# facebookresearch/iris

Hardware: AMD Instinct MI355X
Metric: bake_shading throughput (shading samples/s: secondary rays traced and shaded) (higher is better)
Workload: dtype f32; 1 GPU; bake_shading train-view sequence (15 views evenly spaced among 32 cameras on a circle, one view per step), 1920x1080, SPP=128 per lobe, lobes=[0, 1, 2, 3, 4, 5, 6] (0=diffuse,1-6=specular), synthetic room seed=1 1000990 triangles, SLF H=256, Philox uniforms; pixels_per_view=2073600

## Files before the change

### iris_amd/csrc/iris_bake.h

```cpp
#pragma once
#include "iris_tile.h"

namespace iris {

struct BakeArgs {
    SceneDev sc; EmitDev em; SlfDev slf;
    const float* pos; const float* nrm; const float* wo;
    const float* u2; const int32_t* pix_id;
    int64_t P; int spp; uint64_t seed; uint32_t stream_id; float rough;
    float* out0; float* out1; int64_t* tri_next;
    int64_t* src_next;
    unsigned long long* stats;
    uint32_t* stack_ovf;
    float4* scratch;
    unsigned int* tile_counter;
    int tile_px;
};

#ifndef IRIS_TILE_RAYS
#define IRIS_TILE_RAYS 5120
#endif
constexpr int kTileRays = IRIS_TILE_RAYS;

__device__ __forceinline__ void reduce_geometry(int spp, int& lpp, int& ppw, int& rounds) {
    if (spp >= 64) { lpp = 64; ppw = 1; rounds = (spp + 63) >> 6; }
    else if ((spp & (spp - 1)) == 0) { lpp = spp; ppw = 64 / spp; rounds = 1; }
    else { lpp = 64; ppw = 1; rounds = 1; }
}

struct RayOut { float r0, g0, b0, r1, g1, b1; };

template <bool SPEC>
__device__ __forceinline__ void sample_dir(const BakeArgs& a, float u0, float u1, f3 n, f3 w, f3 t, f3 b, f3& wi, float& g0, float& g1) {
    g0 = 1.f; g1 = 0.f;
    if (SPEC) {
        wi = specular_sampler(u0, u1, a.rough, w, n, t, b);
        SpecW sw = specular_weights(wi, w, n, a.rough, false);
        g0 = sw.g0; g1 = sw.g1;
    } else {
        wi = diffuse_sampler(u0, u1, n, t, b);
    }
}
template <bool SPEC>
__device__ __forceinline__ void sample_lobe(const BakeArgs& a, int64_t p, int s, f3 n, f3 w, f3 t, f3 b, uint64_t base, f3& wi, float& g0, float& g1) {
    float u0, u1;
    if (a.u2) { const float* up = a.u2 + (p * a.spp + s) * 2; u0 = up[0]; u1 = up[1]; }
    else {
        uint32_t s_lo = (uint32_t)a.seed, s_hi = (uint32_t)(a.seed >> 32);
        asm volatile("" : "+s"(s_lo), "+s"(s_hi));
        philox_u2(((uint64_t)s_hi << 32) | s_lo, base + (uint64_t)s, a.stream_id, u0, u1);
    }
    sample_dir<SPEC>(a, u0, u1, n, w, t, b, wi, g0, g1);
}

template <bool SPEC, bool COUNT, int LAYOUT, int LDS_DEPTH = kStackLds, bool GLOBAL_OVF = false>
__device__ __forceinline__ RayOut trace_shade(const BakeArgs& a, int64_t p, int s, f3 x, f3 wi, float g0, float g1, uint32_t* lds_stack,
                                              TraceStats* ts, uint32_t& n_rays, uint32_t* ovf = nullptr) {
    f3 o = mk3(x.x + kRayEps * wi.x, x.y + kRayEps * wi.y, x.z + kRayEps * wi.z);
    const uint32_t steps0 = COUNT ? ts->nodes + ts->tris : 0;
    Hit h = trace_bvh4<LAYOUT, COUNT, LDS_DEPTH, GLOBAL_OVF>(a.sc, o, wi, lds_stack, ts, ovf);
    if (COUNT) {
        n_rays++;
        uint32_t mine = ts->nodes + ts->tris - steps0, mx = mine;
        for (int m = 1; m < 64; m <<= 1) mx = max(mx, (uint32_t)__shfl_xor((int)mx, m));
        if (first_active_lane()) ts->max_steps64 += (unsigned long long)mx * 64ull;
    }
    f3 pn = mk3(0.f, 0.f, 0.f);
    int64_t tri = -1;
    if (h.slot >= 0) {
        f3 p0, p1, p2;
        hit_vertices(a.sc, h, p0, p1, p2);
        pn = hit_position(h, p0, p1, p2);
        tri = h.id;
    }
    if (a.tri_next) a.tri_next[p * a.spp + s] = tri;
    float epdf; bool vn; int src;
    f3 Le = eval_emitter1(a.em, a.slf, pn, tri, true, 1.0f, 0.0f, epdf, vn, src);
    if (a.src_next) a.src_next[p * a.spp + s] = src;
    RayOut r;
    if (SPEC) { r.r0 = Le.x * g0; r.g0 = Le.y * g0; r.b0 = Le.z * g0; r.r1 = Le.x * g1; r.g1 = Le.y * g1; r.b1 = Le.z * g1; }
    else { r.r0 = Le.x; r.g0 = Le.y; r.b0 = Le.z; r.r1 = r.g1 = r.b1 = 0.f; }
    return r;
}

__device__ __forceinline__ bool dead_samples_skippable(const BakeArgs& a) { return !a.tri_next && !a.src_next; }

template <bool SPEC, bool COUNT, int LAYOUT, int LDS_DEPTH = kStackLds, bool GLOBAL_OVF = false>
__device__ __forceinline__ RayOut shade_sample(const BakeArgs& a, int64_t p, int s, f3 x, f3 n, f3 w, f3 t, f3 b, uint64_t base,
                                               uint32_t* lds_stack, TraceStats* ts, uint32_t& n_rays, uint32_t* ovf = nullptr) {
    f3 wi; float g0, g1;
    sample_lobe<SPEC>(a, p, s, n, w, t, b, base, wi, g0, g1);
    if (SPEC && !COUNT && dead_samples_skippable(a) && g0 == 0.f && g1 == 0.f) return RayOut{0.f, 0.f, 0.f, 0.f, 0.f, 0.f};
    return trace_shade<SPEC, COUNT, LAYOUT, LDS_DEPTH, GLOBAL_OVF>(a, p, s, x, wi, g0, g1, lds_stack, ts, n_rays, ovf);
}

template <bool COUNT>
__device__ __forceinline__ void flush_stats(const BakeArgs& a, const TraceStats& ts, uint32_t n_rays) {
    if (COUNT) {
        uint32_t v[8] = {n_rays, ts.nodes, ts.tris, ts.node_iters, ts.leaf_iters, ts.sp_gt8, ts.sp_gt12, ts.sp_gt16};
        for (int k = 0; k < 8; ++k) {
            uint32_t x = v[k];
            for (int m = 1; m < 64; m <<= 1) x += __shfl_xor(x, m);
            if ((threadIdx.x & 63) == 0) atomicAdd(a.stats + k, (unsigned long long)x);
        }
        uint32_t w[2] = {ts.drain_nodes, ts.drain_node_iters};
        for (int k = 0; k < 2; ++k) {
            uint32_t x = w[k];
            for (int m = 1; m < 64; m <<= 1) x += __shfl_xor(x, m);
            if ((threadIdx.x & 63) == 0) atomicAdd(a.stats + 9 + k, (unsigned long long)x);
        }
        uint32_t tp[4] = {ts.top21, ts.top85, ts.top341, ts.top1365};
        for (int k = 0; k < 4; ++k) {
            uint32_t x = tp[k];
            for (int m = 1; m < 64; m <<= 1) x += __shfl_xor(x, m);
            if ((threadIdx.x & 63) == 0) atomicAdd(a.stats + 11 + k, (unsigned long long)x);
        }
        uint32_t sh[5] = {ts.shared_iters, ts.shared_lanes, ts.shared_all_iters, ts.slow_push_iters, ts.shared_path_iters};
        for (int k = 0; k < 5; ++k) {
            uint32_t x = sh[k];
            for (int m = 1; m < 64; m <<= 1) x += __shfl_xor(x, m);
            if ((threadIdx.x & 63) == 0) atomicAdd(a.stats + 15 + k, (unsigned long long)x);
        }
        unsigned long long y = ts.max_steps64;
        for (int m = 1; m < 64; m <<= 1) y += __shfl_xor(y, m);
        if ((threadIdx.x & 63) == 0) atomicAdd(a.stats + 8, y);
    }
}

template <bool SPEC, bool COUNT, int LAYOUT>
__global__ __launch_bounds__(kBlock) void bake_kernel(BakeArgs a) {
    __shared__ uint32_t s_stack[kStackLds * kBlock];
    const int lane = threadIdx.x & 63;
    const int spp = a.spp;
    int lpp, ppw, rounds;
    reduce_geometry(spp, lpp, ppw, rounds);
    const int sub = lane / lpp, sl = lane - sub * lpp;
    const int64_t n_groups = (a.P + ppw - 1) / ppw;
    const int64_t wave0 = ((int64_t)blockIdx.x * kBlock + threadIdx.x) >> 6;
    const int64_t n_waves = ((int64_t)gridDim.x * kBlock) >> 6;
    const float inv_spp = 1.0f / (float)spp;
    TraceStats ts;
    uint32_t n_rays = 0;

    for (int64_t g = wave0; g < n_groups; g += n_waves) {
        const int64_t p = g * ppw + sub;
        const bool pvalid = p < a.P;
        f3 x = mk3(0.f, 0.f, 0.f), n = mk3(0.f, 0.f, 1.f), w = mk3(0.f, 0.f, 1.f), t, b;
        uint64_t base = 0;
        if (pvalid) {
            x = ld3(a.pos + p * 3); n = ld3(a.nrm + p * 3);
            if (SPEC) w = ld3(a.wo + p * 3);
            base = (uint64_t)(a.pix_id ? (int64_t)a.pix_id[p] : p) * (uint64_t)spp;
        }
        normal_space(n, t, b);
        float a0x = 0.f, a0y = 0.f, a0z = 0.f, a1x = 0.f, a1y = 0.f, a1z = 0.f;
        for (int r = 0; r < rounds; ++r) {
            const int s = r * 64 + sl;
            if (pvalid && s < spp) {
                RayOut o = shade_sample<SPEC, COUNT, LAYOUT>(a, p, s, x, n, w, t, b, base, s_stack + threadIdx.x, &ts, n_rays);
                a0x += o.r0; a0y += o.g0; a0z += o.b0;
                if (SPEC) { a1x += o.r1; a1y += o.g1; a1z += o.b1; }
            }
        }
        for (int m = 1; m < lpp; m <<= 1) {
            a0x += __shfl_xor(a0x, m); a0y += __shfl_xor(a0y, m); a0z += __shfl_xor(a0z, m);
            if (SPEC) { a1x += __shfl_xor(a1x, m); a1y += __shfl_xor(a1y, m); a1z += __shfl_xor(a1z, m); }
        }
        if (pvalid && sl == 0) {
            st3(a.out0 + p * 3, mk3(a0x * inv_spp, a0y * inv_spp, a0z * inv_spp));
            if (SPEC) st3(a.out1 + p * 3, mk3(a1x * inv_spp, a1y * inv_spp, a1z * inv_spp));
        }
    }
    flush_stats<COUNT>(a, ts, n_rays);
}

#ifndef IRIS_TILE_WAVES
#define IRIS_TILE_WAVES 7
#endif
#ifndef IRIS_TILE_STACK
#define IRIS_TILE_STACK 12
#endif

template <bool SPEC, bool COUNT, int LAYOUT, int TILE_STACK>
__device__ __forceinline__ void tile_body(const BakeArgs& a, int64_t p0, int np, float4* res, uint16_t* s_sorted, uint32_t* s_stack, int* s_chunk,
                                          uint32_t* ovf, TraceStats& ts, uint32_t& n_rays) {
    const int tid = threadIdx.x, lane = tid & 63, wave = tid >> 6;
    const int spp = a.spp;
    float2* res_g = reinterpret_cast<float2*>(res + kTileRays);
    int lpp, ppw, rounds;
    reduce_geometry(spp, lpp, ppw, rounds);
    const int sub = lane / lpp, sl = lane - sub * lpp;
    const float inv_spp = 1.0f / (float)spp;
    const int nr = np * spp;
    const bool resolve = !a.em.emit_ord && !a.tri_next;
    const bool skip_dead = dead_samples_skippable(a);

    const uint32_t spp_m = spp > 1 ? (uint32_t)(0x100000000ull / (uint64_t)(uint32_t)spp) + 1u : 0u;
    auto div_spp = [&](int r) -> int { return spp > 1 ? (int)__umulhi((uint32_t)r, spp_m) : r; };

    constexpr int kFrameOff = (kTileRays + 2 * 256 * 4) / 4, kFramePx = (TILE_STACK * kBlock - kFrameOff) / 6;
    float* s_frames = reinterpret_cast<float*>(s_stack) + kFrameOff;
    const bool frames = np <= kFramePx;
    if (frames) {
        for (int pl = tid; pl < np; pl += kBlock) {
            f3 t, b;
            normal_space(ld3(a.nrm + (p0 + pl) * 3), t, b);
            float* f = s_frames + pl * 6;
            f[0] = t.x; f[1] = t.y; f[2] = t.z; f[3] = b.x; f[4] = b.y; f[5] = b.z;
        }
        __syncthreads();
    }

    tile_sort_trace<LAYOUT, COUNT, kTileRays, TILE_STACK, true, SPEC && !COUNT>(
        a.sc, nr, s_sorted, s_stack, s_chunk, ovf, ts,
        [&](int r) -> uint32_t {
            const int pl = div_spp(r), s = r - pl * spp;
            const int64_t p = p0 + pl;
            const f3 n = ld3(a.nrm + p * 3), w = SPEC ? ld3(a.wo + p * 3) : mk3(0.f, 0.f, 1.f);
            const uint64_t base = (uint64_t)(a.pix_id ? (int64_t)a.pix_id[p] : p) * (uint64_t)spp;
            f3 t, b;
            if (frames) { const float* f = s_frames + pl * 6; t = mk3(f[0], f[1], f[2]); b = mk3(f[3], f[4], f[5]); }
            else normal_space(n, t, b);
            f3 wi; float g0, g1;
            sample_lobe<SPEC>(a, p, s, n, w, t, b, base, wi, g0, g1);
            if (SPEC) res_g[r] = make_float2(g1, g0);
            const bool dead = SPEC && !COUNT && skip_dead && g0 == 0.f && g1 == 0.f;
            res[r] = dead ? make_float4(0.f, 0.f, __int_as_float(resolve ? 0 : -1), __int_as_float(resolve ? -2 : 0)) : make_float4(wi.x, wi.y, wi.z, 0.f);
            return dead ? kDeadRay : dir_bin(wi);
        },
        [&](int r, f3& o, f3& d) {
            const int64_t p = p0 + div_spp(r);
            o = ld3(a.pos + p * 3);
            const float4 qa = res[r];
            d = mk3(qa.x, qa.y, qa.z);
        },
        [&](f3& o, f3& d) { o = mk3(o.x + kRayEps * d.x, o.y + kRayEps * d.y, o.z + kRayEps * d.z); },
        [&](int r, const Hit& h) {
            if (resolve) {
                float4 q = make_float4(0.f, 0.f, 0.f, __int_as_float(-2));
                if (h.slot >= 0) {
                    const float4* tr = a.sc.tris + (int64_t)h.slot * 4;
                    const float4 tx = tr[0], ty = tr[1], tz = tr[2];
                    const float ow = tr[3].x;
                    const f3 pn = hit_position(h, mk3(tx.x, ty.x, tz.x), mk3(tx.y, ty.y, tz.y), mk3(tx.z, ty.z, tz.z));
                    q = make_float4(pn.x, pn.y, pn.z, ow);
                }
                res[r] = q;
            } else
            res[r] = make_float4(h.u, h.v, __int_as_float(h.slot), 0.f);
            if (COUNT) n_rays++; }
        );

    const int n_groups = (np + ppw - 1) / ppw;
    IRIS_PHASE_BEGIN();
    for (int g = wave; g < n_groups; g += kBlock / 64) {
        const int pl = g * ppw + sub;
        const bool pvalid = pl < np;
        float a0x = 0.f, a0y = 0.f, a0z = 0.f, a1x = 0.f, a1y = 0.f, a1z = 0.f;
        if (resolve) {
            for (int rr = 0; rr < rounds; rr += 2) {
                const int s0 = rr * 64 + sl, s1 = s0 + 64;
                const bool ok0 = pvalid && s0 < spp, ok1 = pvalid && rr + 1 < rounds && s1 < spp;
                float4 q0 = make_float4(0.f, 0.f, 0.f, __int_as_float(-2)), q1 = q0;
                float2 w0 = make_float2(0.f, 0.f), w1 = w0;
                if (ok0) { q0 = res[pl * spp + s0]; if (SPEC) w0 = res_g[pl * spp + s0]; }
                if (ok1) { q1 = res[pl * spp + s1]; if (SPEC) w1 = res_g[pl * spp + s1]; }
                const int o0 = __float_as_int(q0.w), o1 = __float_as_int(q1.w);
                int j0 = -1, j1 = -1;
                if (o0 == -1) j0 = slf_index(a.slf, mk3(q0.x, q0.y, q0.z));
                if (o1 == -1) j1 = slf_index(a.slf, mk3(q1.x, q1.y, q1.z));
                float4 r0 = make_float4(0.f, 0.f, 0.f, 0.f), r1 = r0;
                if (o0 >= 0 || j0 >= 0) r0 = *(o0 >= 0 ? a.em.radiance + o0 : a.slf.radiance + j0);
                if (o1 >= 0 || j1 >= 0) r1 = *(o1 >= 0 ? a.em.radiance + o1 : a.slf.radiance + j1);
                if (ok0) {
                    const float z = o0 >= 0 ? -0.f : 0.f;
                    const f3 Le = mk3(z + r0.x, z + r0.y, z + r0.z);
                    if (a.src_next) a.src_next[(p0 + pl) * spp + s0] = o0 >= 0 ? -2 - o0 : j0;
                    if (SPEC) { a0x += Le.x * w0.y; a0y += Le.y * w0.y; a0z += Le.z * w0.y; a1x += Le.x * w0.x; a1y += Le.y * w0.x; a1z += Le.z * w0.x; }
                    else { a0x += Le.x; a0y += Le.y; a0z += Le.z; }
                }
                if (ok1) {
                    const float z = o1 >= 0 ? -0.f : 0.f;
                    const f3 Le = mk3(z + r1.x, z + r1.y, z + r1.z);
                    if (a.src_next) a.src_next[(p0 + pl) * spp + s1] = o1 >= 0 ? -2 - o1 : j1;
                    if (SPEC) { a0x += Le.x * w1.y; a0y += Le.y * w1.y; a0z += Le.z * w1.y; a1x += Le.x * w1.x; a1y += Le.y * w1.x; a1z += Le.z * w1.x; }
                    else { a0x += Le.x; a0y += Le.y; a0z += Le.z; }
                }
            }
        } else
        for (int rr = 0; rr < rounds; ++rr) {
            const int s = rr * 64 + sl;
            if (pvalid && s < spp) {
                const float4 qa = res[pl * spp + s];
                Hit h; h.u = qa.x; h.v = qa.y; h.slot = __float_as_int(qa.z); h.t = 0.f; h.id = 0;
                f3 pn = mk3(0.f, 0.f, 0.f);
                int64_t tri = -1;
                int ord_rec = -1;
                if (h.slot >= 0) {
                    const float4* tr = a.sc.tris + (int64_t)h.slot * 4;
                    const float4 tx = tr[0], ty = tr[1], tz = tr[2];
                    if (!a.em.emit_ord) ord_rec = __float_as_int(tr[3].x);
                    pn = hit_position(h, mk3(tx.x, ty.x, tz.x), mk3(tx.y, ty.y, tz.y), mk3(tx.z, ty.z, tz.z));
                    tri = __float_as_int(tx.w);
                }
                if (a.tri_next) a.tri_next[(p0 + pl) * spp + s] = tri;
                float epdf; bool vn; int src;
                const f3 Le = eval_emitter1(a.em, a.slf, pn, tri, true, 1.0f, 0.0f, epdf, vn, src, ord_rec);
                if (a.src_next) a.src_next[(p0 + pl) * spp + s] = src;
                if (SPEC) {
                    const float2 qb = res_g[pl * spp + s];
                    a0x += Le.x * qb.y; a0y += Le.y * qb.y; a0z += Le.z * qb.y;
                    a1x += Le.x * qb.x; a1y += Le.y * qb.x; a1z += Le.z * qb.x;
                } else { a0x += Le.x; a0y += Le.y; a0z += Le.z; }
            }
        }
        for (int m = 1; m < lpp; m <<= 1) {
            a0x += __shfl_xor(a0x, m); a0y += __shfl_xor(a0y, m); a0z += __shfl_xor(a0z, m);
            if (SPEC) { a1x += __shfl_xor(a1x, m); a1y += __shfl_xor(a1y, m); a1z += __shfl_xor(a1z, m); }
        }
        if (pvalid && sl == 0) {
            const int64_t p = p0 + pl;
            st3(a.out0 + p * 3, mk3(a0x * inv_spp, a0y * inv_spp, a0z * inv_spp));
            if (SPEC) st3(a.out1 + p * 3, mk3(a1x * inv_spp, a1y * inv_spp, a1z * inv_spp));
        }
    }
    IRIS_PHASE_MARK(3);
}

constexpr int kTileChunk = 64;
__device__ __forceinline__ long long claim_tile(unsigned int* counters, long long n_tiles) {
    constexpr int kChunk = kTileChunk;
    const long long n_chunks = (n_tiles + kChunk - 1) / kChunk;
    for (int k = 0; k < 8; ++k) {
        const int x = ((int)blockIdx.x + k) & 7;
        const long long per = (n_chunks + 7 - x) / 8;
        for (;;) {
            const unsigned int c = atomicAdd(counters + x, 1u);
            const long long ch = (long long)(c / kChunk);
            if (ch >= per) break;
            const long long t = (ch * 8 + x) * kChunk + (c % kChunk);
            if (t < n_tiles) return t;
        }
    }
    return n_tiles;
}

template <bool SPEC, bool COUNT, int LAYOUT>
__global__ __launch_bounds__(kBlock, COUNT ? 4 : IRIS_TILE_WAVES) void bake_tile_kernel(BakeArgs a) {
    constexpr int kTileStack = IRIS_TILE_STACK;
    __shared__ uint16_t s_sorted[kTileRays];
    __shared__ uint32_t s_stack[kTileStack * kBlock];
    __shared__ int s_tile, s_chunk;
    static_assert(kTileStack * kBlock * 4 >= kTileRays + 2 * 256 * 4, "stack region too small to alias the sort keys");
    const int tid = threadIdx.x;
    constexpr int NC = SPEC ? 2 : 1;
    float4* res = a.scratch + (size_t)blockIdx.x * kTileRays * NC;
    uint32_t* ovf = a.stack_ovf + (size_t)blockIdx.x * (kStackCapacity - kTileStack) * kBlock;
    const int64_t n_tiles = (a.P + a.tile_px - 1) / a.tile_px;
    TraceStats ts;
    uint32_t n_rays = 0;
    for (;;) {
        __syncthreads();
        if (tid == 0) { s_tile = (int)claim_tile(a.tile_counter, n_tiles); s_chunk = 0; }
        (s_stack + kTileRays / 4)[tid] = 0;
        __syncthreads();
        const int64_t tile = s_tile;
        if (tile >= n_tiles) break;
        const int64_t p0 = (int64_t)tile * a.tile_px;
        tile_body<SPEC, COUNT, LAYOUT, kTileStack>(a, p0, (int)min((int64_t)a.tile_px, a.P - p0), res, s_sorted, s_stack, &s_chunk, ovf, ts, n_rays);
    }
    flush_stats<COUNT>(a, ts, n_rays);
}

constexpr int kMaxLobes = 8;
struct ViewLobe { float rough; int spp; uint32_t stream_id; int spec; int tile_px; int tiles_per_span; float* out0; float* out1; };
struct ViewArgs {
    BakeArgs base;
    int n_lobes;
    int span_px;
    long long n_tiles;
    ViewLobe lobe[kMaxLobes];
};

template <int LAYOUT>
__global__ __launch_bounds__(kBlock, IRIS_TILE_WAVES) void bake_view_kernel(ViewArgs v) {
    constexpr int kTileStack = IRIS_TILE_STACK;
    __shared__ uint16_t s_sorted[kTileRays];
    __shared__ uint32_t s_stack[kTileStack * kBlock];
    __shared__ int s_tile, s_chunk;
    static_assert(kTileStack * kBlock * 4 >= kTileRays + 2 * 256 * 4, "stack region too small to alias the sort keys");
    const int tid = threadIdx.x;
    float4* res = v.base.scratch + (size_t)blockIdx.x * kTileRays * 2;
    uint32_t* ovf = v.base.stack_ovf + (size_t)blockIdx.x * (kStackCapacity - kTileStack) * kBlock;
    for (;;) {
        __syncthreads();
        if (tid == 0) { s_tile = (int)claim_tile(v.base.tile_counter, v.n_tiles); s_chunk = 0; }
        (s_stack + kTileRays / 4)[tid] = 0;
        __syncthreads();
        const long long vt = s_tile;
        if (vt >= v.n_tiles) break;
        const long long g = vt / kTileChunk, q = g >> 3;
        const int j = (int)(vt % kTileChunk), l = (int)(q % v.n_lobes);
        const int64_t span0 = ((q / v.n_lobes) * 8 + (g & 7)) * (int64_t)v.span_px;
        const int64_t p0 = span0 + (int64_t)j * v.lobe[l].tile_px;
        if (j >= v.lobe[l].tiles_per_span || p0 >= v.base.P) continue;
        const int np = (int)min((int64_t)v.lobe[l].tile_px, min(v.base.P, span0 + v.span_px) - p0);
        BakeArgs a = v.base;
        a.spp = v.lobe[l].spp; a.rough = v.lobe[l].rough; a.stream_id = v.lobe[l].stream_id; a.tile_px = v.lobe[l].tile_px;
        a.out0 = v.lobe[l].out0; a.out1 = v.lobe[l].out1; a.u2 = nullptr; a.tri_next = nullptr; a.src_next = nullptr;
        TraceStats ts; uint32_t n_rays = 0;
        if (v.lobe[l].spec) tile_body<true, false, LAYOUT, kTileStack>(a, p0, np, res, s_sorted, s_stack, &s_chunk, ovf, ts, n_rays);
        else tile_body<false, false, LAYOUT, kTileStack>(a, p0, np, res, s_sorted, s_stack, &s_chunk, ovf, ts, n_rays);
    }
}

}
```

### iris_amd/csrc/iris_tile.h

```cpp
#pragma once
#include "iris_trace.h"

namespace iris {

#ifndef IRIS_PRIO_A
#define IRIS_PRIO_A 0
#endif
#ifndef IRIS_PRIO_C
#define IRIS_PRIO_C 3
#endif
#ifndef IRIS_PRIO_D
#define IRIS_PRIO_D 0
#endif

__device__ __forceinline__ uint32_t dir_bin(f3 d) {
    const float ax = fabsf(d.x), ay = fabsf(d.y), az = fabsf(d.z);
    const float inv = __builtin_amdgcn_rcpf(ax + ay + az + 1e-30f);
    const float a = ax * inv, b = ay * inv;
    const float v = b * __builtin_amdgcn_rcpf(1.f - a + 1e-30f);
    const int iu = min(7, (int)(a * 8.f)), iv0 = min(3, (int)(v * 4.f));
    const int iv = (iu & 1) ? 3 - iv0 : iv0;
    const uint32_t oct = (d.x < 0.f ? 1u : 0u) | (d.y < 0.f ? 2u : 0u) | (d.z < 0.f ? 4u : 0u);
    return (oct << 5) | ((uint32_t)iu << 2) | (uint32_t)iv;
}

#ifdef IRIS_PHASE_TIMING
__device__ unsigned long long g_phase_cycles[8];
#define IRIS_PHASE_BEGIN() unsigned long long t_phase_ = clock64()
#define IRIS_PHASE_MARK(k) do { if (threadIdx.x == 0) { const unsigned long long t_ = clock64(); atomicAdd(&g_phase_cycles[k], t_ - t_phase_); t_phase_ = t_; } } while (0)
#else
#define IRIS_PHASE_BEGIN()
#define IRIS_PHASE_MARK(k)
#endif

constexpr uint32_t kDeadRay = 256u;
template <int LAYOUT, bool COUNT, int CAP, int TILE_STACK, bool GLOBAL_OVF, bool SKIP_DEAD = false, class PhaseA, class FetchRay, class Prepare, class Retire>
__device__ __forceinline__ void tile_sort_trace(const SceneDev& sc, int nr, uint16_t* s_sorted, uint32_t* s_stack, int* s_chunk, uint32_t* ovf,
                                                TraceStats& ts, PhaseA phase_a, FetchRay fetch_ray, Prepare prepare, Retire retire) {
    static_assert(TILE_STACK * kBlock * 4 >= CAP + 2 * 256 * 4, "stack region too small to alias the sort keys");
    static_assert(!SKIP_DEAD || CAP <= 32 * kBlock, "one bit per ray of a thread");
    uint8_t* s_keys = reinterpret_cast<uint8_t*>(s_stack);
    uint32_t* s_hist = s_stack + CAP / 4;
    uint32_t* s_cur = s_hist + 256;
    const int tid = threadIdx.x, lane = tid & 63, wave = tid >> 6;
    IRIS_PHASE_BEGIN();
    __builtin_amdgcn_s_setprio(IRIS_PRIO_A);
    uint32_t dead = 0;
    if (SKIP_DEAD) {
        uint32_t bit = 1u;
        for (int r = tid; r < nr; r += kBlock, bit <<= 1) {
            const uint32_t key = phase_a(r);
            if (key == kDeadRay) dead |= bit;
            else { s_keys[r] = (uint8_t)key; atomicAdd(&s_hist[key], 1u); }
        }
    } else
    for (int r = tid; r < nr; r += kBlock) {
        const uint32_t key = phase_a(r);
        s_keys[r] = (uint8_t)key;
        atomicAdd(&s_hist[key], 1u);
    }
    __syncthreads();
    IRIS_PHASE_MARK(0);
    if (wave == 0) {
        uint32_t c0 = s_hist[lane * 4], c1 = s_hist[lane * 4 + 1], c2 = s_hist[lane * 4 + 2], c3 = s_hist[lane * 4 + 3];
        uint32_t tot = c0 + c1 + c2 + c3, inc = tot;
        for (int m = 1; m < 64; m <<= 1) { uint32_t v = __shfl_up(inc, m); if (lane >= m) inc += v; }
        uint32_t ex = inc - tot;
        if (SKIP_DEAD) {
            const uint32_t first = (uint32_t)nr - (uint32_t)__builtin_amdgcn_readlane((int)inc, 63);
            ex += first;
            if (lane == 0) *s_chunk = (int)first;
        }
        s_cur[lane * 4] = ex; s_cur[lane * 4 + 1] = ex + c0; s_cur[lane * 4 + 2] = ex + c0 + c1; s_cur[lane * 4 + 3] = ex + c0 + c1 + c2;
    }
    __syncthreads();
    if (SKIP_DEAD) {
        for (int r = tid; r < nr; r += kBlock, dead >>= 1) {
            if (dead & 1u) continue;
            const uint32_t pos = atomicAdd(&s_cur[s_keys[r]], 1u);
            s_sorted[pos] = (uint16_t)r;
        }
    } else
    for (int r = tid; r < nr; r += kBlock) {
        const uint32_t pos = atomicAdd(&s_cur[s_keys[r]], 1u);
        s_sorted[pos] = (uint16_t)r;
    }
    __syncthreads();
    IRIS_PHASE_MARK(1);
    {
        int my_r = 0;
        auto fetch = [&](f3& o, f3& d) -> bool {
            const unsigned long long m = __ballot(1);
            int base = 0;
            if (lane == __ffsll((long long)m) - 1) base = atomicAdd(s_chunk, __popcll(m));
            base = __builtin_amdgcn_readfirstlane(base);
            const int i = base + (int)__builtin_amdgcn_mbcnt_hi((uint32_t)(m >> 32), __builtin_amdgcn_mbcnt_lo((uint32_t)m, 0u));
            if (i >= nr) return false;
            my_r = s_sorted[i];
            fetch_ray(my_r, o, d);
            return true;
        };
        auto ret = [&](const Hit& h) { retire(my_r, h); };
        __builtin_amdgcn_s_setprio(IRIS_PRIO_C);
        uint32_t tid_c = threadIdx.x;
        asm volatile("" : "+v"(tid_c));
        SceneDev sc_c = sc;
        asm volatile("" : "+s"(sc_c.nodes), "+s"(sc_c.tris), "+s"(sc_c.oct_stride));
        trace_stream<LAYOUT, COUNT, TILE_STACK, GLOBAL_OVF>(sc_c, s_stack + tid_c, tid_c, ovf, &ts, fetch, prepare, ret);
        __builtin_amdgcn_s_setprio(IRIS_PRIO_D);
        IRIS_PHASE_MARK(4);
    }
    __syncthreads();
    IRIS_PHASE_MARK(2);
}

}
```

Before: 10510 Mrays/s.

## Reload kernel arguments per phase to shrink live scalar register state

Restructures tile_body so each phase (sampling, tracing, shading) reloads only the kernel arguments it needs straight from the kernarg segment via fresh pointers, instead of holding a full BakeArgs copy live across the whole tile. The goal is to cut SGPR/VGPR pressure and spills across the long trace loop, which could allow more waves or a tighter inner loop. Adds lobe-source abstractions for the single-lobe and multi-lobe view kernels. The cost is repeated scalar loads from kernarg memory at each phase entry, and the changes depend on compiler register allocation behaving as intended.

```diff
diff --git a/iris_amd/csrc/iris_bake.h b/iris_amd/csrc/iris_bake.h
--- a/iris_amd/csrc/iris_bake.h
+++ b/iris_amd/csrc/iris_bake.h
@@ -30,8 +30,8 @@
 
 struct RayOut { float r0, g0, b0, r1, g1, b1; };
 
-template <bool SPEC>
-__device__ __forceinline__ void sample_dir(const BakeArgs& a, float u0, float u1, f3 n, f3 w, f3 t, f3 b, f3& wi, float& g0, float& g1) {
+template <bool SPEC, class A>
+__device__ __forceinline__ void sample_dir(const A& a, float u0, float u1, f3 n, f3 w, f3 t, f3 b, f3& wi, float& g0, float& g1) {
     g0 = 1.f; g1 = 0.f;
     if (SPEC) {
         wi = specular_sampler(u0, u1, a.rough, w, n, t, b);
@@ -41,8 +41,8 @@
         wi = diffuse_sampler(u0, u1, n, t, b);
     }
 }
-template <bool SPEC>
-__device__ __forceinline__ void sample_lobe(const BakeArgs& a, int64_t p, int s, f3 n, f3 w, f3 t, f3 b, uint64_t base, f3& wi, float& g0, float& g1) {
+template <bool SPEC, class A>
+__device__ __forceinline__ void sample_lobe(const A& a, int64_t p, int s, f3 n, f3 w, f3 t, f3 b, uint64_t base, f3& wi, float& g0, float& g1) {
     float u0, u1;
     if (a.u2) { const float* up = a.u2 + (p * a.spp + s) * 2; u0 = up[0]; u1 = up[1]; }
     else {
@@ -181,75 +181,172 @@
 #define IRIS_TILE_STACK 12
 #endif
 
-template <bool SPEC, bool COUNT, int LAYOUT, int TILE_STACK>
-__device__ __forceinline__ void tile_body(const BakeArgs& a, int64_t p0, int np, float4* res, uint16_t* s_sorted, uint32_t* s_stack, int* s_chunk,
-                                          uint32_t* ovf, TraceStats& ts, uint32_t& n_rays) {
-    const int tid = threadIdx.x, lane = tid & 63, wave = tid >> 6;
-    const int spp = a.spp;
-    float2* res_g = reinterpret_cast<float2*>(res + kTileRays);
-    int lpp, ppw, rounds;
-    reduce_geometry(spp, lpp, ppw, rounds);
-    const int sub = lane / lpp, sl = lane - sub * lpp;
-    const float inv_spp = 1.0f / (float)spp;
+constexpr int kMaxLobes = 8;
+struct ViewLobe { float rough; int spp; uint32_t stream_id; int spec; int tile_px; int tiles_per_span; float* out0; float* out1; };
+struct ViewArgs {
+    BakeArgs base;
+    int n_lobes;
+    int span_px;
+    long long n_tiles;
+    ViewLobe lobe[kMaxLobes];
+};
+
+typedef const __attribute__((address_space(4))) BakeArgs karg_bake;
+typedef const __attribute__((address_space(4))) ViewArgs karg_view;
+static_assert(offsetof(ViewArgs, base) == 0, "the view kernel's arguments start with the BakeArgs the tile phases read");
+__device__ __forceinline__ karg_bake* kernarg_fresh() {
+    karg_bake* k = (karg_bake*)__builtin_amdgcn_kernarg_segment_ptr();
+    asm volatile("" : "+s"(k));
+    return k;
+}
+template <bool SPEC>
+struct TileLobeSrc {
+    static constexpr int kSlabSlots = SPEC ? 2 : 1;
+    __device__ __forceinline__ float rough(karg_bake* k) const { return k->rough; }
+    __device__ __forceinline__ uint32_t stream_id(karg_bake* k) const { return k->stream_id; }
+    __device__ __forceinline__ float* out0(karg_bake* k) const { return k->out0; }
+    __device__ __forceinline__ float* out1(karg_bake* k) const { return k->out1; }
+    __device__ __forceinline__ const float* u2(karg_bake* k) const { return k->u2; }
+    __device__ __forceinline__ int64_t* tri_next(karg_bake* k) const { return k->tri_next; }
+    __device__ __forceinline__ int64_t* src_next(karg_bake* k) const { return k->src_next; }
+};
+struct ViewLobeSrc {
+    static constexpr int kSlabSlots = 2;
+    int l;
+    __device__ __forceinline__ const __attribute__((address_space(4))) ViewLobe* lobe(karg_bake* k) const { return ((karg_view*)k)->lobe + l; }
+    __device__ __forceinline__ float rough(karg_bake* k) const { return lobe(k)->rough; }
+    __device__ __forceinline__ uint32_t stream_id(karg_bake* k) const { return lobe(k)->stream_id; }
+    __device__ __forceinline__ float* out0(karg_bake* k) const { return lobe(k)->out0; }
+    __device__ __forceinline__ float* out1(karg_bake* k) const { return lobe(k)->out1; }
+    __device__ __forceinline__ const float* u2(karg_bake*) const { return nullptr; }
+    __device__ __forceinline__ int64_t* tri_next(karg_bake*) const { return nullptr; }
+    __device__ __forceinline__ int64_t* src_next(karg_bake*) const { return nullptr; }
+};
+template <class LOBE>
+__device__ __forceinline__ float4* tile_slab(karg_bake* k) { return k->scratch + (size_t)blockIdx.x * kTileRays * LOBE::kSlabSlots; }
+template <int TILE_STACK>
+__device__ __forceinline__ uint32_t* tile_ovf(karg_bake* k) { return k->stack_ovf + (size_t)blockIdx.x * (kStackCapacity - TILE_STACK) * kBlock; }
+
+struct SampleView {
+    const float* nrm; const float* wo; const int32_t* pix_id; const float* u2;
+    uint64_t seed; uint32_t stream_id; float rough; int spp; uint32_t spp_m;
+    float4* res;
+    bool resolve, skip_dead;
+};
+struct TraceView {
+    SceneDev sc;
+    const float* pos; float4* res; uint32_t* ovf;
+    int spp; uint32_t spp_m;
+    bool resolve;
+};
+struct ShadeView {
+    EmitDev em; SlfDev slf;
+    const float4* tris;
+    float4* res; float* out0; float* out1; int64_t* tri_next; int64_t* src_next;
+};
+
+template <bool SPEC, bool COUNT, int LAYOUT, int TILE_STACK, class LOBE>
+__device__ __forceinline__ void tile_body(const LOBE lobe, int64_t p0, int np, int spp, uint16_t* s_sorted, uint32_t* s_stack, int* s_chunk,
+                                          TraceStats& ts, uint32_t& n_rays) {
+    const int tid = threadIdx.x;
     const int nr = np * spp;
-    const bool resolve = !a.em.emit_ord && !a.tri_next;
-    const bool skip_dead = dead_samples_skippable(a);
 
     const uint32_t spp_m = spp > 1 ? (uint32_t)(0x100000000ull / (uint64_t)(uint32_t)spp) + 1u : 0u;
-    auto div_spp = [&](int r) -> int { return spp > 1 ? (int)__umulhi((uint32_t)r, spp_m) : r; };
+    auto div_spp = [](int r, int spp_c, uint32_t m) -> int { return spp_c > 1 ? (int)__umulhi((uint32_t)r, m) : r; };
 
     constexpr int kFrameOff = (kTileRays + 2 * 256 * 4) / 4, kFramePx = (TILE_STACK * kBlock - kFrameOff) / 6;
     float* s_frames = reinterpret_cast<float*>(s_stack) + kFrameOff;
     const bool frames = np <= kFramePx;
-    if (frames) {
-        for (int pl = tid; pl < np; pl += kBlock) {
-            f3 t, b;
-            normal_space(ld3(a.nrm + (p0 + pl) * 3), t, b);
-            float* f = s_frames + pl * 6;
-            f[0] = t.x; f[1] = t.y; f[2] = t.z; f[3] = b.x; f[4] = b.y; f[5] = b.z;
-        }
-        __syncthreads();
-    }
-
+
+    SampleView sv;
+    TraceView tv;
     tile_sort_trace<LAYOUT, COUNT, kTileRays, TILE_STACK, true, SPEC && !COUNT>(
-        a.sc, nr, s_sorted, s_stack, s_chunk, ovf, ts,
+        tv.sc, nr, s_sorted, s_stack, s_chunk, tv.ovf, ts,
         [&](int r) -> uint32_t {
-            const int pl = div_spp(r), s = r - pl * spp;
+            const int pl = div_spp(r, sv.spp, sv.spp_m), s = r - pl * sv.spp;
             const int64_t p = p0 + pl;
-            const f3 n = ld3(a.nrm + p * 3), w = SPEC ? ld3(a.wo + p * 3) : mk3(0.f, 0.f, 1.f);
-            const uint64_t base = (uint64_t)(a.pix_id ? (int64_t)a.pix_id[p] : p) * (uint64_t)spp;
+            const f3 n = ld3(sv.nrm + p * 3), w = SPEC ? ld3(sv.wo + p * 3) : mk3(0.f, 0.f, 1.f);
+            const uint64_t base = (uint64_t)(sv.pix_id ? (int64_t)sv.pix_id[p] : p) * (uint64_t)sv.spp;
             f3 t, b;
             if (frames) { const float* f = s_frames + pl * 6; t = mk3(f[0], f[1], f[2]); b = mk3(f[3], f[4], f[5]); }
             else normal_space(n, t, b);
             f3 wi; float g0, g1;
-            sample_lobe<SPEC>(a, p, s, n, w, t, b, base, wi, g0, g1);
-            if (SPEC) res_g[r] = make_float2(g1, g0);
-            const bool dead = SPEC && !COUNT && skip_dead && g0 == 0.f && g1 == 0.f;
-            res[r] = dead ? make_float4(0.f, 0.f, __int_as_float(resolve ? 0 : -1), __int_as_float(resolve ? -2 : 0)) : make_float4(wi.x, wi.y, wi.z, 0.f);
+            sample_lobe<SPEC>(sv, p, s, n, w, t, b, base, wi, g0, g1);
+            if (SPEC) reinterpret_cast<float2*>(sv.res + kTileRays)[r] = make_float2(g1, g0);
+            const bool dead = SPEC && !COUNT && sv.skip_dead && g0 == 0.f && g1 == 0.f;
+            sv.res[r] = dead ? make_float4(0.f, 0.f, __int_as_float(sv.resolve ? 0 : -1), __int_as_float(sv.resolve ? -2 : 0)) : make_float4(wi.x, wi.y, wi.z, 0.f);
             return dead ? kDeadRay : dir_bin(wi);
         },
         [&](int r, f3& o, f3& d) {
-            const int64_t p = p0 + div_spp(r);
-            o = ld3(a.pos + p * 3);
-            const float4 qa = res[r];
+            const int64_t p = p0 + div_spp(r, tv.spp, tv.spp_m);
+            o = ld3(tv.pos + p * 3);
+            const float4 qa = tv.res[r];
             d = mk3(qa.x, qa.y, qa.z);
         },
         [&](f3& o, f3& d) { o = mk3(o.x + kRayEps * d.x, o.y + kRayEps * d.y, o.z + kRayEps * d.z); },
         [&](int r, const Hit& h) {
-            if (resolve) {
+            if (tv.resolve) {
                 float4 q = make_float4(0.f, 0.f, 0.f, __int_as_float(-2));
                 if (h.slot >= 0) {
-                    const float4* tr = a.sc.tris + (int64_t)h.slot * 4;
+                    const float4* tr = tv.sc.tris + (int64_t)h.slot * 4;
                     const float4 tx = tr[0], ty = tr[1], tz = tr[2];
                     const float ow = tr[3].x;
                     const f3 pn = hit_position(h, mk3(tx.x, ty.x, tz.x), mk3(tx.y, ty.y, tz.y), mk3(tx.z, ty.z, tz.z));
                     q = make_float4(pn.x, pn.y, pn.z, ow);
                 }
-                res[r] = q;
+                tv.res[r] = q;
             } else
-            res[r] = make_float4(h.u, h.v, __int_as_float(h.slot), 0.f);
-            if (COUNT) n_rays++; }
-        );
+            tv.res[r] = make_float4(h.u, h.v, __int_as_float(h.slot), 0.f);
+            if (COUNT) n_rays++; },
+        [&]() {
+            karg_bake* k = kernarg_fresh();
+            sv.nrm = k->nrm; sv.wo = k->wo; sv.pix_id = k->pix_id; sv.u2 = lobe.u2(k);
+            sv.seed = k->seed; sv.stream_id = lobe.stream_id(k); sv.rough = lobe.rough(k);
+            sv.spp = spp; sv.spp_m = spp_m;
+            asm volatile("" : "+s"(sv.spp), "+s"(sv.spp_m));
+            sv.res = tile_slab<LOBE>(k);
+            const bool ids = lobe.tri_next(k) != nullptr;
+            sv.resolve = !k->em.emit_ord && !ids;
+            sv.skip_dead = !ids && !lobe.src_next(k);
+            if (frames) {
+                for (int pl = tid; pl < np; pl += kBlock) {
+                    f3 t, b;
+                    normal_space(ld3(sv.nrm + (p0 + pl) * 3), t, b);
+                    float* f = s_frames + pl * 6;
+                    f[0] = t.x; f[1] = t.y; f[2] = t.z; f[3] = b.x; f[4] = b.y; f[5] = b.z;
+                }
+                __syncthreads();
+            }
+        },
+        [&]() {
+            karg_bake* k = kernarg_fresh();
+            tv.sc.nodes = k->sc.nodes; tv.sc.tris = k->sc.tris; tv.sc.n_nodes = 0; tv.sc.n_tris = 0;
+            tv.sc.phase_min = k->sc.phase_min; tv.sc.layout = LAYOUT; tv.sc.oct_stride = k->sc.oct_stride;
+            tv.pos = k->pos; tv.res = tile_slab<LOBE>(k); tv.ovf = tile_ovf<TILE_STACK>(k);
+            tv.spp = spp; tv.spp_m = spp_m;
+            asm volatile("" : "+s"(tv.spp), "+s"(tv.spp_m));
+            tv.resolve = !k->em.emit_ord && !lobe.tri_next(k);
+        });
+
+    ShadeView dv;
+    {
+        karg_bake* k = kernarg_fresh();
+        dv.em.emit_ord = k->em.emit_ord; dv.em.radiance = k->em.radiance; dv.em.area = k->em.area; dv.em.nf = k->em.nf; dv.em.emitter_pdf = k->em.emitter_pdf;
+        dv.slf.inds = k->slf.inds; dv.slf.radiance = k->slf.radiance; dv.slf.H = k->slf.H; dv.slf.vmin = k->slf.vmin; dv.slf.den = k->slf.den;
+        dv.tris = k->sc.tris;
+        dv.res = tile_slab<LOBE>(k); dv.out0 = lobe.out0(k); dv.out1 = lobe.out1(k); dv.tri_next = lobe.tri_next(k); dv.src_next = lobe.src_next(k);
+    }
+    const ShadeView& a = dv;
+    uint32_t tid_d = threadIdx.x;
+    asm volatile("" : "+v"(tid_d));
+    const int lane = (int)(tid_d & 63u), wave = (int)(tid_d >> 6);
+    float4* const res = dv.res;
+    float2* const res_g = reinterpret_cast<float2*>(res + kTileRays);
+    const bool resolve = !a.em.emit_ord && !a.tri_next;
+    int lpp, ppw, rounds;
+    reduce_geometry(spp, lpp, ppw, rounds);
+    const int sub = lane / lpp, sl = lane - sub * lpp;
+    const float inv_spp = 1.0f / (float)spp;
 
     const int n_groups = (np + ppw - 1) / ppw;
     IRIS_PHASE_BEGIN();
@@ -297,7 +394,7 @@
                 int64_t tri = -1;
                 int ord_rec = -1;
                 if (h.slot >= 0) {
-                    const float4* tr = a.sc.tris + (int64_t)h.slot * 4;
+                    const float4* tr = a.tris + (int64_t)h.slot * 4;
                     const float4 tx = tr[0], ty = tr[1], tz = tr[2];
                     if (!a.em.emit_ord) ord_rec = __float_as_int(tr[3].x);
                     pn = hit_position(h, mk3(tx.x, ty.x, tz.x), mk3(tx.y, ty.y, tz.y), mk3(tx.z, ty.z, tz.z));
@@ -353,34 +450,24 @@
     __shared__ int s_tile, s_chunk;
     static_assert(kTileStack * kBlock * 4 >= kTileRays + 2 * 256 * 4, "stack region too small to alias the sort keys");
     const int tid = threadIdx.x;
-    constexpr int NC = SPEC ? 2 : 1;
-    float4* res = a.scratch + (size_t)blockIdx.x * kTileRays * NC;
-    uint32_t* ovf = a.stack_ovf + (size_t)blockIdx.x * (kStackCapacity - kTileStack) * kBlock;
-    const int64_t n_tiles = (a.P + a.tile_px - 1) / a.tile_px;
     TraceStats ts;
     uint32_t n_rays = 0;
     for (;;) {
+        karg_bake* k = kernarg_fresh();
+        const int64_t P = k->P;
+        const int tile_px = k->tile_px;
+        const int64_t n_tiles = (P + tile_px - 1) / tile_px;
         __syncthreads();
-        if (tid == 0) { s_tile = (int)claim_tile(a.tile_counter, n_tiles); s_chunk = 0; }
+        if (tid == 0) { s_tile = (int)claim_tile(k->tile_counter, n_tiles); s_chunk = 0; }
         (s_stack + kTileRays / 4)[tid] = 0;
         __syncthreads();
         const int64_t tile = s_tile;
         if (tile >= n_tiles) break;
-        const int64_t p0 = (int64_t)tile * a.tile_px;
-        tile_body<SPEC, COUNT, LAYOUT, kTileStack>(a, p0, (int)min((int64_t)a.tile_px, a.P - p0), res, s_sorted, s_stack, &s_chunk, ovf, ts, n_rays);
+        const int64_t p0 = (int64_t)tile * tile_px;
+        tile_body<SPEC, COUNT, LAYOUT, kTileStack>(TileLobeSrc<SPEC>{}, p0, (int)min((int64_t)tile_px, P - p0), k->spp, s_sorted, s_stack, &s_chunk, ts, n_rays);
     }
     flush_stats<COUNT>(a, ts, n_rays);
 }
-
-constexpr int kMaxLobes = 8;
-struct ViewLobe { float rough; int spp; uint32_t stream_id; int spec; int tile_px; int tiles_per_span; float* out0; float* out1; };
-struct ViewArgs {
-    BakeArgs base;
-    int n_lobes;
-    int span_px;
-    long long n_tiles;
-    ViewLobe lobe[kMaxLobes];
-};
 
 template <int LAYOUT>
 __global__ __launch_bounds__(kBlock, IRIS_TILE_WAVES) void bake_view_kernel(ViewArgs v) {
@@ -390,28 +477,29 @@
     __shared__ int s_tile, s_chunk;
     static_assert(kTileStack * kBlock * 4 >= kTileRays + 2 * 256 * 4, "stack region too small to alias the sort keys");
     const int tid = threadIdx.x;
-    float4* res = v.base.scratch + (size_t)blockIdx.x * kTileRays * 2;
-    uint32_t* ovf = v.base.stack_ovf + (size_t)blockIdx.x * (kStackCapacity - kTileStack) * kBlock;
     for (;;) {
+        karg_view* kv = (karg_view*)kernarg_fresh();
+        const long long n_tiles = kv->n_tiles;
         __syncthreads();
-        if (tid == 0) { s_tile = (int)claim_tile(v.base.tile_counter, v.n_tiles); s_chunk = 0; }
+        if (tid == 0) { s_tile = (int)claim_tile(kv->base.tile_counter, n_tiles); s_chunk = 0; }
         (s_stack + kTileRays / 4)[tid] = 0;
         __syncthreads();
         const long long vt = s_tile;
-        if (vt >= v.n_tiles) break;
+        if (vt >= n_tiles) break;
+        const int n_lobes = kv->n_lobes, span_px = kv->span_px;
+        const int64_t P = kv->base.P;
         const long long g = vt / kTileChunk, q = g >> 3;
-        const int j = (int)(vt % kTileChunk), l = (int)(q % v.n_lobes);
-        const int64_t span0 = ((q / v.n_lobes) * 8 + (g & 7)) * (int64_t)v.span_px;
-        const int64_t p0 = span0 + (int64_t)j * v.lobe[l].tile_px;
-        if (j >= v.lobe[l].tiles_per_span || p0 >= v.base.P) continue;
-        const int np = (int)min((int64_t)v.lobe[l].tile_px, min(v.base.P, span0 + v.span_px) - p0);
-        BakeArgs a = v.base;
-        a.spp = v.lobe[l].spp; a.rough = v.lobe[l].rough; a.stream_id = v.lobe[l].stream_id; a.tile_px = v.lobe[l].tile_px;
-        a.out0 = v.lobe[l].out0; a.out1 = v.lobe[l].out1; a.u2 = nullptr; a.tri_next = nullptr; a.src_next = nullptr;
+        const int j = (int)(vt % kTileChunk), l = (int)(q % n_lobes);
+        const int tile_px = kv->lobe[l].tile_px;
+        const int64_t span0 = ((q / n_lobes) * 8 + (g & 7)) * (int64_t)span_px;
+        const int64_t p0 = span0 + (int64_t)j * tile_px;
+        if (j >= kv->lobe[l].tiles_per_span || p0 >= P) continue;
+        const int np = (int)min((int64_t)tile_px, min(P, span0 + span_px) - p0);
+        const int spp = kv->lobe[l].spp;
         TraceStats ts; uint32_t n_rays = 0;
-        if (v.lobe[l].spec) tile_body<true, false, LAYOUT, kTileStack>(a, p0, np, res, s_sorted, s_stack, &s_chunk, ovf, ts, n_rays);
-        else tile_body<false, false, LAYOUT, kTileStack>(a, p0, np, res, s_sorted, s_stack, &s_chunk, ovf, ts, n_rays);
-    }
-}
-
-}
+        if (kv->lobe[l].spec) tile_body<true, false, LAYOUT, kTileStack>(ViewLobeSrc{l}, p0, np, spp, s_sorted, s_stack, &s_chunk, ts, n_rays);
+        else tile_body<false, false, LAYOUT, kTileStack>(ViewLobeSrc{l}, p0, np, spp, s_sorted, s_stack, &s_chunk, ts, n_rays);
+    }
+}
+
+}
diff --git a/iris_amd/csrc/iris_tile.h b/iris_amd/csrc/iris_tile.h
--- a/iris_amd/csrc/iris_tile.h
+++ b/iris_amd/csrc/iris_tile.h
@@ -34,15 +34,19 @@
 #endif
 
 constexpr uint32_t kDeadRay = 256u;
-template <int LAYOUT, bool COUNT, int CAP, int TILE_STACK, bool GLOBAL_OVF, bool SKIP_DEAD = false, class PhaseA, class FetchRay, class Prepare, class Retire>
-__device__ __forceinline__ void tile_sort_trace(const SceneDev& sc, int nr, uint16_t* s_sorted, uint32_t* s_stack, int* s_chunk, uint32_t* ovf,
-                                                TraceStats& ts, PhaseA phase_a, FetchRay fetch_ray, Prepare prepare, Retire retire) {
+struct NoPhaseHook { __device__ __forceinline__ void operator()() const {} };
+template <int LAYOUT, bool COUNT, int CAP, int TILE_STACK, bool GLOBAL_OVF, bool SKIP_DEAD = false, class PhaseA, class FetchRay, class Prepare, class Retire,
+          class EnterA = NoPhaseHook, class EnterC = NoPhaseHook>
+__device__ __forceinline__ void tile_sort_trace(const SceneDev& sc, int nr, uint16_t* s_sorted, uint32_t* s_stack, int* s_chunk, uint32_t* const& ovf,
+                                                TraceStats& ts, PhaseA phase_a, FetchRay fetch_ray, Prepare prepare, Retire retire,
+                                                EnterA enter_a = EnterA(), EnterC enter_c = EnterC()) {
     static_assert(TILE_STACK * kBlock * 4 >= CAP + 2 * 256 * 4, "stack region too small to alias the sort keys");
     static_assert(!SKIP_DEAD || CAP <= 32 * kBlock, "one bit per ray of a thread");
     uint8_t* s_keys = reinterpret_cast<uint8_t*>(s_stack);
     uint32_t* s_hist = s_stack + CAP / 4;
     uint32_t* s_cur = s_hist + 256;
     const int tid = threadIdx.x, lane = tid & 63, wave = tid >> 6;
+    enter_a();
     IRIS_PHASE_BEGIN();
     __builtin_amdgcn_s_setprio(IRIS_PRIO_A);
     uint32_t dead = 0;
@@ -88,6 +92,7 @@
     __syncthreads();
     IRIS_PHASE_MARK(1);
     {
+        enter_c();
         int my_r = 0;
         auto fetch = [&](f3& o, f3& d) -> bool {
             const unsigned long long m = __ballot(1);
```

Result: no change. 10560 Mrays/s (median of 6 runs) (+0.5%).
